# spaceandtimefdn/blitzar

Hardware: NVIDIA H100
Metric: MSM throughput (scalar*point terms/sec), ristretto255, n=2^20 per GPU (higher is better)
Workload: dtype u32 limbs (integer modular arithmetic)

## Files before the change

blitzar_b200/csrc/msm.cuh:

```cuda
#pragma once
#include <algorithm>
#include <vector>

#include "batch_affine.cuh"
#include "curve.cuh"
#include "engine_api.cuh"
#include "lanefield.cuh"

namespace b200 {

struct ColumnDesc {
  const unsigned char* base;
  u64 row_stride;
  u32 bit_offset;
  u32 bit_width;
  u32 n;
  u32 is_signed;
  u32 first_window;
  u32 num_windows;
  u32 table_n;
  u32 gen_base;
};
B200_HD u32 bucket_windows(const ColumnDesc& col) { return col.table_n ? (col.num_windows ? 1u : 0u) : col.num_windows; }

B200_HD void load_scalar_bits(u32 v[8], bool& negative, const ColumnDesc& col, u64 i) {
  const unsigned char* row = col.base + i * col.row_stride;
#pragma unroll
  for (int k = 0; k < 8; ++k)
    v[k] = 0;
  const u32 width = col.bit_width;
  const unsigned char* p = row + (col.bit_offset >> 3);
  const u32 sh = col.bit_offset & 7u;
  if (sh == 0 && width == 256 && (((size_t)p) & 15u) == 0) {
    const uint4* q = (const uint4*)p;
    uint4 a = q[0], b = q[1];
    v[0] = a.x; v[1] = a.y; v[2] = a.z; v[3] = a.w;
    v[4] = b.x; v[5] = b.y; v[6] = b.z; v[7] = b.w;
  } else if (sh == 0 && (width & 31u) == 0 && (((size_t)p) & 3u) == 0) {
    const u32* q = (const u32*)p;
#pragma unroll
    for (int k = 0; k < 8; ++k)
      if ((u32)k < (width >> 5))
        v[k] = q[k];
  } else {
    const u32 nbytes = (sh + width + 7u) >> 3;
#pragma unroll
    for (int k = 0; k < 8; ++k) {
      u64 acc = 0;
#pragma unroll
      for (int b = 0; b < 5; ++b) {
        u32 idx = 4u * k + b;
        if (idx < nbytes)
          acc |= (u64)p[idx] << (8 * b);
      }
      v[k] = (u32)(acc >> sh);
    }
#pragma unroll
    for (int k = 0; k < 8; ++k) {
      int lo = 32 * k;
      if ((int)width <= lo)
        v[k] = 0;
      else if ((int)width < lo + 32)
        v[k] &= (1u << (width - lo)) - 1u;
    }
  }
  negative = false;
  if (col.is_signed) {
    u32 top = width - 1;
    bool neg = false;
#pragma unroll
    for (int k = 0; k < 8; ++k)
      if ((top >> 5) == (u32)k)
        neg = (v[k] >> (top & 31u)) & 1u;
    if (neg) {
      u64 c = 1;
#pragma unroll
      for (int k = 0; k < 8; ++k) {
        int lo = 32 * k;
        u32 m = 0;
        if ((int)width >= lo + 32)
          m = 0xffffffffu;
        else if ((int)width > lo)
          m = (1u << (width - lo)) - 1u;
        c += (u64)((~v[k]) & m);
        v[k] = (u32)c & m;
        c = (m == 0xffffffffu) ? (c >> 32) : 0;
      }
      negative = true;
    }
  }
}

constexpr u32 kAllWindows = 0xffffffffu;
template <class Fn>
B200_HD void for_each_digit(const u32 v[8], bool negative, const ColumnDesc& col, u32 c,
                            u32 nbuckets, Fn f, u32 only_window = kAllWindows) {
  const u32 half = nbuckets;
  const u32 mask = (1u << c) - 1u;
  u64 buf = 0;
  u32 nb = 0, w = 0, carry = 0;
  const u32 W = only_window == kAllWindows
                    ? col.num_windows
                    : (only_window < col.num_windows ? only_window + 1 : 0u);
#pragma unroll
  for (int k = 0; k < 8; ++k) {
    buf |= (u64)v[k] << nb;
    nb += 32;
    while (nb >= c && w < W) {
      u32 d = ((u32)buf & mask) + carry;
      buf >>= c;
      nb -= c;
      bool dneg = d > half;
      carry = dneg ? 1u : 0u;
      if (dneg)
        d = (1u << c) - d;
      if (d && (only_window == kAllWindows || w == only_window))
        f((col.first_window + (col.table_n ? 0u : w)) * nbuckets + (d - 1u), negative != dneg, w);
      ++w;
    }
  }
  while (w < W) {
    u32 d = ((u32)buf & mask) + carry;
    buf >>= c;
    bool dneg = d > half;
    carry = dneg ? 1u : 0u;
    if (dneg)
      d = (1u << c) - d;
    if (d && (only_window == kAllWindows || w == only_window))
      f((col.first_window + (col.table_n ? 0u : w)) * nbuckets + (d - 1u), negative != dneg, w);
    ++w;
  }
}

B200_HD u32 column_of(const u64* col_start, u32 ncols, u64 tid) {
  u32 lo = 0, hi = ncols;
  while (hi - lo > 1) {
    const u32 mid = (lo + hi) >> 1;
    if (tid >= col_start[mid])
      lo = mid;
    else
      hi = mid;
  }
  return lo;
}
struct CountBody {
  static constexpr int kBlock = 256;
  const ColumnDesc* cols;
  const u64* col_start;
  u32 ncols, c, nbuckets;
  u32* counts;
  B200_HD void operator()(u64 tid) const {
    const u32 j = column_of(col_start, ncols, tid);
    const ColumnDesc col = cols[j];
    u64 i = tid - col_start[j];
    u32 v[8];
    bool neg;
    load_scalar_bits(v, neg, col, i);
    u32* cnt = counts;
    for_each_digit(v, neg, col, c, nbuckets, [cnt](u32 key, bool, u32) { B200_ATOMIC_ADD(&cnt[key], 1u); });
  }
};

struct ScatterBody {
  static constexpr int kBlock = 256;
  const ColumnDesc* cols;
  const u64* col_start;
  u32 ncols, c, nbuckets;
  u32* cursor;
  u64* entries;
  u64 total_terms;
  B200_HD void operator()(u64 tid) const {
    u32 only = kAllWindows;
    if (total_terms) {
      only = (u32)(tid / total_terms);
      tid -= (u64)only * total_terms;
    }
    const u32 j = column_of(col_start, ncols, tid);
    const ColumnDesc col = cols[j];
    if (only != kAllWindows && only >= col.num_windows)
      return;
    u64 i = tid - col_start[j];
    u32 v[8];
    bool neg;
    load_scalar_bits(v, neg, col, i);
    u32* cur = cursor;
    u64* en = entries;
    const u32 ii = (u32)i + col.gen_base, tn = col.table_n;
    for_each_digit(v, neg, col, c, nbuckets, [cur, en, ii, tn](u32 key, bool negate, u32 w) {
      u32 pos = B200_ATOMIC_ADD(&cur[key], 1u);
      en[pos] = ((u64)key << 32) | (u64)(((ii + w * tn) << 1) | (negate ? 1u : 0u));
    }, only);
  }
};

constexpr u32 kScanChunk = 256, kScanChunkFirst = 64;
struct ScanUpBody {
  static constexpr int kBlock = 128;
  const u32* in;
  u64 n;
  u32* partial;
  u32 chunk;
  B200_HD void operator()(u64 t) const {
    u64 b = t * chunk, e = b + chunk < n ? b + chunk : n;
    u32 s = 0;
    for (u64 i = b; i < e; ++i)
      s += in[i];
    partial[t] = s;
  }
};
struct ScanTopBody {
  static constexpr int kBlock = 32;
  u32* data;
  u64 n;
  B200_HD void operator()(u64) const {
    u32 s = 0;
    for (u64 i = 0; i < n; ++i) {
      u32 v = data[i];
      data[i] = s;
      s += v;
    }
  }
};
struct ScanDownBody {
  static constexpr int kBlock = 128;
  u32* data;
  u64 n;
  const u32* partial_scanned;
  u32 chunk;
  B200_HD void operator()(u64 t) const {
    u64 b = t * chunk, e = b + chunk < n ? b + chunk : n;
    u32 s = partial_scanned[t];
    for (u64 i = b; i < e; ++i) {
      u32 v = data[i];
      data[i] = s;
      s += v;
    }
  }
};

inline void exclusive_scan(u32* data, u64 n, stream_t s, u32 chunk = kScanChunkFirst) {
  if (n <= kScanChunk) {
    launch(ScanTopBody{data, n}, 1, s);
    return;
  }
  u64 m = (n + chunk - 1) / chunk;
  u32* partial = (u32*)dev_alloc(m * sizeof(u32), s);
  launch(ScanUpBody{data, n, partial, chunk}, m, s);
  exclusive_scan(partial, m, s, kScanChunk);
  launch(ScanDownBody{data, n, partial, chunk}, m, s);
  dev_free(partial, s);
}

#if defined(__CUDACC__) && !defined(B200_EMULATE)
#define B200_BINNED_SORT 1
constexpr u32 kMicroBins = 16384, kBinCap = 8192, kBinSpan = 4096, kMaxBinShift = 12;
constexpr u64 kBinnedSortMinEntries = 1ull << 20;

template <int kBlock> __device__ u32 block_exclusive_scan(u32 v, u32* warp_sums, u32* total) {
  const u32 lane = threadIdx.x & 31u, warp = threadIdx.x >> 5;
  u32 x = v;
#pragma unroll
  for (int d = 1; d < 32; d <<= 1) {
    const u32 y = __shfl_up_sync(0xffffffffu, x, d);
    if (lane >= (u32)d)
      x += y;
  }
  if (lane == 31)
    warp_sums[warp] = x;
  __syncthreads();
  if (warp == 0) {
    u32 w = lane < kBlock / 32 ? warp_sums[lane] : 0u;
#pragma unroll
    for (int d = 1; d < 32; d <<= 1) {
      const u32 y = __shfl_up_sync(0xffffffffu, w, d);
      if (lane >= (u32)d)
        w += y;
    }
    if (lane < kBlock / 32)
      warp_sums[lane] = w;
  }
  __syncthreads();
  const u32 pre = (warp ? warp_sums[warp - 1] : 0u) + x - v;
  *total = warp_sums[kBlock / 32 - 1];
  __syncthreads();
  return pre;
}

template <class Fn>
__device__ void for_each_entry(const ColumnDesc* cols, const u64* col_start, u32 ncols, u32 c,
                               u32 nbuckets, u64 tid, Fn f) {
  const u32 j = column_of(col_start, ncols, tid);
  const ColumnDesc col = cols[j];
  const u64 i = tid - col_start[j];
  u32 v[8];
  bool neg;
  load_scalar_bits(v, neg, col, i);
  const u32 ii = (u32)i + col.gen_base, tn = col.table_n;
  for_each_digit(v, neg, col, c, nbuckets, [&](u32 key, bool negate, u32 w) {
    f(key, ((u64)key << 32) | (u64)(((ii + w * tn) << 1) | (negate ? 1u : 0u)));
  });
}

struct MicroCountBody {
  static constexpr int kBlock = 512;
  const ColumnDesc* cols;
  const u64* col_start;
  u32 ncols, c, nbuckets;
  u64 total_terms;
  u32 tile, shift, nmicro;
  u32* micro_counts;
  __device__ void run(u32 b, unsigned char* smem) const {
    u32* h = (u32*)smem;
    for (u32 m = threadIdx.x; m < nmicro; m += kBlock)
      h[m] = 0;
    __syncthreads();
    const u64 lo = (u64)b * tile, hi = lo + tile < total_terms ? lo + tile : total_terms;
    const u32 sh = shift;
    for (u64 t = lo + threadIdx.x; t < hi; t += kBlock)
      for_each_entry(cols, col_start, ncols, c, nbuckets, t,
                     [h, sh](u32 key, u64) { atomicAdd(&h[key >> sh], 1u); });
    __syncthreads();
    for (u32 m = threadIdx.x; m < nmicro; m += kBlock)
      if (h[m])
        atomicAdd(&micro_counts[m], h[m]);
  }
};

struct PlanBinsBody {
  static constexpr int kBlock = 1024;
  const u32* micro_counts;
  u32 nmicro, span_micro;
  u64 nkeys;
  u32* bin_of;
  u32* bin_start;
  u32* bin_micro;
  u32* bin_cursor;
  u32* nbins_out;
  u32* counts;
  u32* d_m;
  __device__ bool starts_bin(const u32* st, u32 m) const {
    constexpr u32 H = kBinCap / 2;
    return m == 0 || m % span_micro == 0 || micro_counts[m] > H || micro_counts[m - 1] > H ||
           st[m] / H != st[m - 1] / H;
  }
  __device__ void run(u32, unsigned char* smem) const {
    __shared__ u32 ws[32];
    u32* st = (u32*)smem;
    const u32 per = (nmicro + kBlock - 1) / kBlock, m0 = min(threadIdx.x * per, nmicro),
              m1 = min(m0 + per, nmicro);
    u32 sum = 0;
    for (u32 m = m0; m < m1; ++m)
      sum += micro_counts[m];
    u32 total;
    u32 run = block_exclusive_scan<kBlock>(sum, ws, &total);
    for (u32 m = m0; m < m1; ++m) {
      st[m] = run;
      run += micro_counts[m];
    }
    __syncthreads();
    u32 nf = 0;
    for (u32 m = m0; m < m1; ++m)
      nf += starts_bin(st, m) ? 1u : 0u;
    u32 nbins;
    u32 id = block_exclusive_scan<kBlock>(nf, ws, &nbins);
    for (u32 m = m0; m < m1; ++m) {
      if (starts_bin(st, m)) {
        bin_start[id] = st[m];
        bin_micro[id] = m;
        bin_cursor[id] = st[m];
        ++id;
      }
      bin_of[m] = id - 1;
    }
    if (threadIdx.x == 0) {
      bin_start[nbins] = total;
      bin_micro[nbins] = nmicro;
      *nbins_out = nbins;
      counts[nkeys] = total;
      d_m[0] = total;
    }
  }
};

struct CoarseScatterBody {
  static constexpr int kBlock = 1024;
  const ColumnDesc* cols;
  const u64* col_start;
  u32 ncols, c, nbuckets;
  u64 total_terms;
  u32 tile, shift, nmicro;
  const u32* bin_of;
  const u32* nbins_ptr;
  u32* bin_cursor;
  u64* tmp;
  __device__ void run(u32 b, unsigned char* smem) const {
    __shared__ u32 ws[32];
    u32* h = (u32*)smem;
    u32* delta = h + nmicro;
    u64* stage = (u64*)(delta + nmicro + (nmicro & 1u));
    const u32 nbins = *nbins_ptr;
    for (u32 k = threadIdx.x; k < nbins; k += kBlock)
      h[k] = 0;
    __syncthreads();
    const u64 lo = (u64)b * tile, hi = lo + tile < total_terms ? lo + tile : total_terms;
    const u32 sh = shift;
    const u32* map = bin_of;
    for (u64 t = lo + threadIdx.x; t < hi; t += kBlock)
      for_each_entry(cols, col_start, ncols, c, nbuckets, t,
                     [h, sh, map](u32 key, u64) { atomicAdd(&h[__ldg(&map[key >> sh])], 1u); });
    __syncthreads();
    const u32 per = (nbins + kBlock - 1) / kBlock, k0 = min(threadIdx.x * per, nbins),
              k1 = min(k0 + per, nbins);
    u32 sum = 0;
    for (u32 k = k0; k < k1; ++k)
      sum += h[k];
    u32 size;
    u32 run = block_exclusive_scan<kBlock>(sum, ws, &size);
    for (u32 k = k0; k < k1; ++k) {
      const u32 n = h[k];
      if (n)
        delta[k] = atomicAdd(&bin_cursor[k], n) - run;
      h[k] = run;
      run += n;
    }
    __syncthreads();
    for (u64 t = lo + threadIdx.x; t < hi; t += kBlock)
      for_each_entry(cols, col_start, ncols, c, nbuckets, t, [h, sh, map, stage](u32 key, u64 e) {
        stage[atomicAdd(&h[__ldg(&map[key >> sh])], 1u)] = e;
      });
    __syncthreads();
    for (u32 i = threadIdx.x; i < size; i += kBlock) {
      const u64 e = stage[i];
      tmp[delta[__ldg(&map[(u32)(e >> 32) >> sh])] + i] = e;
    }
  }
};

struct BinSortBody {
  static constexpr int kBlock = 1024;
  static constexpr size_t kSmem = 2 * kBinCap * sizeof(u64) + kBinSpan * sizeof(u32);
  const u64* tmp;
  const u32* bin_start;
  const u32* bin_micro;
  const u32* nbins_ptr;
  u32 shift;
  u64 nkeys;
  u64* entries;
  u32* counts;
  __device__ void run(u32 b, unsigned char* smem) const {
    __shared__ u32 ws[32];
    if (b >= *nbins_ptr)
      return;
    u64* ent = (u64*)smem;
    u32* h = (u32*)(smem + 2 * kBinCap * sizeof(u64));
    const u32 lo = bin_start[b], size = bin_start[b + 1] - lo;
    const u64 klo = (u64)bin_micro[b] << shift, khi_m = (u64)bin_micro[b + 1] << shift;
    const u32 span = (u32)((khi_m < nkeys ? khi_m : nkeys) - klo);
    const bool local = size <= kBinCap;
    for (u32 k = threadIdx.x; k < span; k += kBlock)
      h[k] = 0;
    if (local) {
#pragma unroll 4
      for (u32 i = threadIdx.x; i < size; i += kBlock)
        ent[i] = tmp[(u64)lo + i];
    }
    __syncthreads();
    for (u32 i = threadIdx.x; i < size; i += kBlock) {
      const u64 e = local ? ent[i] : tmp[(u64)lo + i];
      atomicAdd(&h[(u32)(e >> 32) - (u32)klo], 1u);
    }
    __syncthreads();
    const u32 per = (span + kBlock - 1) / kBlock, k0 = min(threadIdx.x * per, span),
              k1 = min(k0 + per, span);
    u32 sum = 0;
    for (u32 k = k0; k < k1; ++k)
      sum += h[k];
    u32 total;
    u32 run = block_exclusive_scan<kBlock>(sum, ws, &total);
    for (u32 k = k0; k < k1; ++k) {
      const u32 n = h[k];
      h[k] = run;
      run += n;
      counts[klo + k] = lo + run;
    }
    __syncthreads();
    if (!local) {
      for (u32 i = threadIdx.x; i < size; i += kBlock) {
        const u64 e = tmp[(u64)lo + i];
        entries[(u64)lo + atomicAdd(&h[(u32)(e >> 32) - (u32)klo], 1u)] = e;
      }
      return;
    }
    u64* sorted = ent + kBinCap;
    for (u32 i = threadIdx.x; i < size; i += kBlock) {
      const u64 e = ent[i];
      sorted[atomicAdd(&h[(u32)(e >> 32) - (u32)klo], 1u)] = e;
    }
    __syncthreads();
    for (u32 i = threadIdx.x; i < size; i += kBlock)
      entries[(u64)lo + i] = sorted[i];
  }
};

inline u32 binned_sort_shift(u64 nkeys) {
  u32 shift = 0;
  while ((nkeys + (1ull << shift) - 1) >> shift > kMicroBins)
    ++shift;
  return shift;
}

inline void binned_sort(stream_t s, const ColumnDesc* d_cols, const u64* d_col_start, u32 ncols,
                        u32 c, u32 nbuckets, u64 total_terms, u64 max_entries, u32 max_windows,
                        u64 nkeys, u64* entries, u32* counts, u32* d_m) {
  const u32 shift = binned_sort_shift(nkeys);
  const u32 nmicro = (u32)((nkeys + (1ull << shift) - 1) >> shift);
  const u32 span_micro = std::max(1u, kBinSpan >> shift);
  u32* ws = (u32*)dev_alloc((5ull * nmicro + 3) * sizeof(u32), s);
  u32 *micro_counts = ws, *bin_of = ws + nmicro, *bin_cursor = ws + 2ull * nmicro,
      *bin_start = ws + 3ull * nmicro, *bin_micro = ws + 4ull * nmicro + 1,
      *nbins = ws + 5ull * nmicro + 2;
  u64* tmp = (u64*)dev_alloc(std::max<u64>(max_entries, 1) * sizeof(u64), s);
  dev_zero(micro_counts, nmicro * sizeof(u32), s);
  const u64 count_tile = 4096;
  launch_blocks(MicroCountBody{d_cols, d_col_start, ncols, c, nbuckets, total_terms,
                               (u32)count_tile, shift, nmicro, micro_counts},
                (total_terms + count_tile - 1) / count_tile, nmicro * sizeof(u32), s);
  launch_blocks(PlanBinsBody{micro_counts, nmicro, span_micro, nkeys, bin_of, bin_start, bin_micro,
                             bin_cursor, nbins, counts, d_m},
                1, nmicro * sizeof(u32), s);
  const size_t scatter_smem = 220 * 1024;
  const size_t bin_bytes = (2ull * nmicro + 2) * sizeof(u32);
  const u64 stage_entries = (scatter_smem - bin_bytes) / sizeof(u64);
  const u64 scatter_tile = std::max<u64>(1, stage_entries / max_windows);
  launch_blocks(CoarseScatterBody{d_cols, d_col_start, ncols, c, nbuckets, total_terms,
                                  (u32)scatter_tile, shift, nmicro, bin_of, nbins, bin_cursor, tmp},
                (total_terms + scatter_tile - 1) / scatter_tile, scatter_smem, s);
  launch_blocks(BinSortBody{tmp, bin_start, bin_micro, nbins, shift, nkeys, entries, counts}, nmicro,
                BinSortBody::kSmem, s);
  dev_free(tmp, s);
  dev_free(ws, s);
}
#endif

template <class C> struct FillIdentityBody {
  static constexpr int kBlock = 256;
  static constexpr u32 kChunks = sizeof(typename C::Point) / 16;
  static_assert(sizeof(typename C::Point) % 16 == 0, "points are made of 16-byte aligned fields");
  uint4* p;
  B200_HD void operator()(u64 t) const {
    const typename C::Point id = C::identity();
    const u32 k = (u32)(t % kChunks);
    uint4 v = ((const uint4*)&id)[0];
#pragma unroll
    for (u32 j = 1; j < kChunks; ++j)
      if (j == k)
        v = ((const uint4*)&id)[j];
    p[t] = v;
  }
};
template <class C> inline void fill_identity(stream_t s, typename C::Point* p, u64 n) {
  launch(FillIdentityBody<C>{(uint4*)p}, n * FillIdentityBody<C>::kChunks, s);
}

template <class C> struct MergeBucketsBody {
  static constexpr int kBlock = 128;
  const u32* bucket_end;
  const u32* bucket_begin;
  const typename C::Point* scratch;
  typename C::Point* buckets;
  B200_HD void operator()(u64 k) const {
    const u32 lo = bucket_begin ? bucket_begin[k] : (k ? bucket_end[k - 1] : 0u);
    if (bucket_end[k] == lo)
      return;
    typename C::Point b = buckets[k];
    C::add(b, b, scratch[k]);
    buckets[k] = b;
  }
};

template <class C, bool kGather, class X = SeqExec, bool kUniform = false, bool kUnitZ = false>
struct AccumulateBody {
  static constexpr int kBlock = 128;
  static constexpr int kMinBlocks = !kGather ? 1 : (C::F::N > 8 ? 2 : 3);
  typedef typename C::Point Point;
  typedef typename C::Gen Gen;
  const u32* keys;
  const u64* entries;
  const Gen* gens;
  const Point* pieces;
  const u32* m_ptr;
  u32 K;
  u32 final_level;
  Point* buckets;
  u32* out_keys;
  Point* out_pieces;
  u32* out_m_ptr;
  const u32* unit_veto;

  B200_HD void put_bucket(u32 key, const Point& acc, bool writer) const {
    if (writer)
      buckets[key] = acc;
  }
  B200_HD u32 key_at(u64 i) const { return kGather ? (u32)(entries[i] >> 32) : keys[i]; }
  B200_HD void fetch(Point& acc, u64 i, bool first) const {
    if (kGather) {
      u32 e = (u32)entries[i];
      if (first)
        C::gen_to_point(acc, gens[e >> 1], e & 1u);
      else
        C::template add_gen<X>(acc, acc, gens[e >> 1], e & 1u);
    } else {
      if (first)
        acc = pieces[i];
      else
        C::template add<X>(acc, acc, pieces[i]);
    }
  }
  template <bool kUnit> B200_HD Gen load_gen(u32 idx) const {
    if constexpr (kUnit)
      return C::load_unit_gen(gens + idx);
    else
      return gens[idx];
  }
  template <bool kUnit>
  B200_HD void gather_walk(u64 t, u64 b, u64 e, bool writer, u32& cur, Point& acc,
                           bool& first_seg) const {
    u64 ent = entries[b];
    Gen g = load_gen<kUnit>((u32)ent >> 1);
    cur = (u32)(ent >> 32);
    struct {
      Point p;
      B200_HD void start(const Gen& g, bool negate) { C::gen_to_point(p, g, negate); }
      B200_HD void add(const Gen& g, bool negate) {
        C::template add_gen<X>(p, p, g, negate, kUnit);
      }
      B200_HD void get(Point& out) const { out = p; }
    } ga;
    for (u64 i = b; i < e; ++i) {
      u64 ent_n = ent;
      Gen g_n = g;
      if (i + 1 < e) {
        ent_n = entries[i + 1];
        g_n = load_gen<kUnit>((u32)ent_n >> 1);
      }
      const u32 k = (u32)(ent >> 32);
      const bool negate = ((u32)ent & 1u) != 0;
      if (kUniform) {
        if (i == b) {
          ga.p = C::identity();
        } else if (k != cur) {
          ga.get(acc);
          if (final_level || !first_seg) {
            put_bucket(cur, acc, writer);
          } else if (writer) {
            out_keys[2 * t] = cur;
            out_pieces[2 * t] = acc;
          }
          first_seg = false;
          cur = k;
          ga.p = C::identity();
        }
        ga.add(g, negate);
      } else if (i == b) {
        ga.start(g, negate);
      } else if (k == cur) {
        ga.add(g, negate);
      } else {
        ga.get(acc);
        if (final_level || !first_seg) {
          put_bucket(cur, acc, writer);
        } else if (writer) {
          out_keys[2 * t] = cur;
          out_pieces[2 * t] = acc;
        }
        first_seg = false;
        cur = k;
        ga.start(g, negate);
      }
      ent = ent_n;
      g = g_n;
    }
    ga.get(acc);
  }
  B200_HD void operator()(u64 tid) const {
    const u64 t = tid / X::kLanes;
    const bool writer = (tid % X::kLanes) == 0;
    const u64 M = *m_ptr;
    const u64 T = (M + K - 1) / K;
    if (tid == 0 && out_m_ptr)
      *out_m_ptr = final_level ? 0u : (u32)(2 * T);
    u64 b = t * K;
    if (b >= M)
      return;
    u64 e = b + K < M ? b + K : M;
    u32 cur;
    Point acc;
    bool first_seg = true;
    if (kGather) {
      if (kUnitZ && unit_veto && *unit_veto)
        gather_walk<false>(t, b, e, writer, cur, acc, first_seg);
      else
        gather_walk<kUnitZ>(t, b, e, writer, cur, acc, first_seg);
    } else {
      cur = key_at(b);
      fetch(acc, b, true);
      for (u64 i = b + 1; i < e; ++i) {
        u32 k = key_at(i);
        if (k == cur) {
          fetch(acc, i, false);
        } else {
          if (final_level || !first_seg) {
            put_bucket(cur, acc, writer);
          } else if (writer) {
            out_keys[2 * t] = cur;
            out_pieces[2 * t] = acc;
          }
          first_seg = false;
          cur = k;
          fetch(acc, i, true);
        }
      }
    }
    if (final_level) {
      put_bucket(cur, acc, writer);
      return;
    }
    if (!writer)
      return;
    if (first_seg) {
      out_keys[2 * t] = cur;
      out_pieces[2 * t] = acc;
      out_keys[2 * t + 1] = cur;
      out_pieces[2 * t + 1] = C::identity();
    } else {
      out_keys[2 * t + 1] = cur;
      out_pieces[2 * t + 1] = acc;
    }
  }
};

struct WindowUsedBody {
  static constexpr int kBlock = 64;
  const u32* bucket_end;
  u32 nbuckets;
  u32* window_used;
  B200_HD void operator()(u64 w) const {
    u32 lo = w ? bucket_end[w * nbuckets - 1] : 0u;
    u32 hi = bucket_end[(w + 1) * nbuckets - 1];
    if (hi != lo)
      window_used[w] = 1u;
  }
};

struct WindowUsedFromCountsBody {
  static constexpr int kBlock = 128;
  const u32* counts;
  u64 nkeys;
  u32 nbuckets;
  u32* window_used;
  B200_HD void operator()(u64 t) const {
    const u64 b = t * 256, e = b + 256 < nkeys ? b + 256 : nkeys;
    for (u64 k = b; k < e; ++k)
      if (counts[k])
        window_used[k / nbuckets] = 1u;
  }
};

template <class C, class Ex = SeqExec> struct ReduceBody {
  static constexpr int kBlock = 64;
  typedef typename C::Point Point;
  const Point* X;
  const Point* Cin;
  u32 m_in, g, log2g;
  Point* Xout;
  Point* Cout;
  const u32* window_used;
  u32 nbuckets;
  B200_HD void operator()(u64 tid) const {
    const u64 t = tid / Ex::kLanes;
    const bool writer = (tid % Ex::kLanes) == 0;
    const u32 m_out = m_in / g;
    const u32 w = (u32)(t / m_out), k = (u32)(t % m_out);
    if (window_used[w] == 0) {
      if (writer) {
        Xout[t] = C::identity();
        Cout[t] = C::identity();
      }
      return;
    }
    const Point* x = X + (u64)w * m_in + (u64)k * g;
    Point run = x[g - 1];
    Point acc = Cin ? C::identity() : run;
    if (Cin) {
      acc = run;
      if (g == 1)
        acc = C::identity();
    }
    for (u32 r = g - 1; r-- > 0;) {
      C::template add<Ex>(run, run, x[r]);
      if (r > 0 || !Cin)
        C::template add<Ex>(acc, acc, run);
    }
    if (Cin) {
      const Point* cin = Cin + (u64)w * m_in + (u64)k * g;
      for (u32 r = 0; r < g; ++r)
        C::template add<Ex>(acc, acc, cin[r]);
    }
    for (u32 i = 0; i < log2g; ++i)
      C::template dbl<Ex>(run, run);
    if (writer) {
      Xout[t] = run;
      Cout[t] = acc;
    }
  }
};

template <class C, class X = SeqExec> struct CombineBody {
  static constexpr int kBlock = 32;
  typedef typename C::Point Point;
  const Point* S;
  const ColumnDesc* cols;
  u32 c;
  Point* out;
  B200_HD void operator()(u64 tid) const {
    const u64 j = tid / X::kLanes;
    const bool writer = (tid % X::kLanes) == 0;
    const ColumnDesc col = cols[j];
    if (col.num_windows == 0 || col.n == 0) {
      if (writer)
        out[j] = C::identity();
      return;
    }
    const u32 nw = bucket_windows(col);
    Point acc = S[col.first_window + nw - 1];
    for (u32 w = nw - 1; w-- > 0;) {
      for (u32 i = 0; i < c; ++i)
        C::template dbl<X>(acc, acc);
      C::template add<X>(acc, acc, S[col.first_window + w]);
    }
    if (writer)
      out[j] = acc;
  }
};

#if defined(__CUDACC__) && !defined(B200_EMULATE)
#define B200_LANE_TAIL 1
struct CombineLaneBody {
  static constexpr int kBlock = 32;
  typedef Ed25519 C;
  const C::Point* S;
  const ColumnDesc* cols;
  u32 c;
  C::Point* out;
  __device__ void operator()(u64 tid) const {
    const u64 j = tid >> 5;
    const ColumnDesc col = cols[j];
    if (col.num_windows == 0 || col.n == 0) {
      if ((tid & 31u) == 0)
        out[j] = C::identity();
      return;
    }
    const lane10::Lane L = lane10::lane_info();
    const u32 nw = bucket_windows(col);
    C::Point acc = S[col.first_window + nw - 1];
    for (u32 w = nw - 1; w-- > 0;) {
      u32 t;
      const u32 v = lane10::dbl_n(L, lane10::slice_point(L, acc), (int)c, t);
      lane10::gather_point(acc, v, t);
      C::add<QuadExecConv>(acc, acc, S[col.first_window + w]);
    }
    if ((tid & 31u) == 0)
      out[j] = acc;
  }
};
struct LanePow {
  static __device__ __forceinline__ void pow22523(F25519::E& r, const F25519::E& a) {
    const lane10::Lane L = lane10::lane_info();
    const u32 g = L.base / 10u;
    lane10::gather(r, lane10::pow22523(L, lane10::slice(L, a)), g < 3 ? g : 0u);
  }
};
struct StoreLaneBody {
  static constexpr int kBlock = 32;
  const Ed25519::Point* pts;
  unsigned char* out;
  u64 count;
  __device__ void operator()(u64 tid) const {
    const u32 lane = (u32)tid & 31u, g = lane / 10u;
    const u64 i = (tid >> 5) * 3 + g;
    const bool live = g < 3 && i < count;
    unsigned char enc[32];
    Ed25519::encode<LanePow>(enc, pts[live ? i : count - 1]);
    if (live && lane == 10u * g) {
      uint4* d = (uint4*)(out + 32 * i);
      const uint4* e = (const uint4*)enc;
      d[0] = e[0];
      d[1] = e[1];
    }
  }
};
#endif

template <class C>
inline void launch_store_commit(stream_t s, const typename C::Point* pts, unsigned char* out,
                                u64 count, bool lane_tail = true);

template <class C, bool kProjective> struct IngestBody {
  static constexpr int kBlock = 128;
  const unsigned char* raw;
  typename C::Gen* gens;
  B200_HD void operator()(u64 i) const {
    typename C::Gen g;
    if (kProjective)
      C::load_proj_abi(g, raw + i * C::kAbiProjBytes);
    else
      C::load_gen_abi(g, raw + i * C::kAbiGenBytes);
    gens[i] = g;
  }
};
constexpr int kMaxTableWindows = 33;
template <class C> struct PrecomputeTableBody {
  static constexpr int kBlock = 64;
  typename C::Gen* table;
  u64 n;
  u32 c, W;
  B200_HD void operator()(u64 i) const {
    typedef typename C::F F;
    typename C::Point p, pts[kMaxTableWindows];
    typename F::E prefix[kMaxTableWindows], acc = F::one(), inv;
    C::gen_to_point(p, table[i], false);
    for (u32 w = 0; w < W; ++w) {
      if (w)
        for (u32 k = 0; k < c; ++k)
          C::dbl(p, p);
      pts[w] = p;
      prefix[w] = acc;
      F::mul(acc, acc, C::denominator(p));
    }
    F::invert(inv, acc);
    for (u32 w = W; w-- > 0;) {
      typename F::E zi;
      F::mul(zi, inv, prefix[w]);
      F::mul(inv, inv, C::denominator(pts[w]));
      typename C::Gen g;
      C::normalized_gen(g, pts[w], zi);
      table[(u64)w * n + i] = g;
    }
  }
};
template <class C> struct IngestCompactBody {
  static constexpr int kBlock = 128;
  const unsigned char* table;
  u32 window_width;
  typename C::Gen* gens;
  B200_HD void operator()(u64 i) const {
    const u64 group = i / window_width, j = i % window_width;
    const u64 entry = (group << window_width) + (1ull << j);
    typename C::Gen g;
    C::load_compact_abi(g, table + entry * C::kAbiCompactBytes);
    gens[i] = g;
  }
};
struct BuiltinGeneratorBody {
  static constexpr int kBlock = 64;
  Ed25519::Gen* gens;
  u64 first;
  B200_HD void operator()(u64 i) const {
    Ed25519::Point g;
    Ed25519::builtin_generator(g, first + i);
    Ed25519::point_to_gen(gens[i], g);
  }
};
struct GenPieces {
  const u64* start;
  const u64* from;
  const u64* to;
  u32 npieces;
};
template <class C> struct IngestPiecesBody {
  static constexpr int kBlock = IngestBody<C, false>::kBlock;
  const unsigned char* raw;
  typename C::Gen* gens;
  GenPieces p;
  B200_HD void operator()(u64 tid) const {
    const u32 k = column_of(p.start, p.npieces, tid);
    IngestBody<C, false>{raw + p.from[k] * C::kAbiGenBytes, gens + p.to[k]}(tid - p.start[k]);
  }
};
struct BuiltinPiecesBody {
  static constexpr int kBlock = BuiltinGeneratorBody::kBlock;
  Ed25519::Gen* gens;
  GenPieces p;
  B200_HD void operator()(u64 tid) const {
    const u32 k = column_of(p.start, p.npieces, tid);
    BuiltinGeneratorBody{gens + p.to[k], p.from[k]}(tid - p.start[k]);
  }
};

struct IngestMap {
  GenPieces p;
  B200_HD void at(u64 i, u64& src, u64& dst) const {
    if (p.npieces == 0) {
      src = dst = i;
      return;
    }
    const u32 k = column_of(p.start, p.npieces, i);
    src = p.from[k] + (i - p.start[k]);
    dst = p.to[k] + (i - p.start[k]);
  }
};
constexpr u32 kNormBlock = 256;
struct NormalizeUpBody {
  static constexpr int kBlock = 128;
  typedef F25519 F;
  const unsigned char* raw;
  IngestMap map;
  u64 n, T;
  F::E* pre;
  F::E* prod;
  u32* invalid;
  B200_HD F::E group(u64 j) const {
    F::E z[kBatchGroup], acc = F::one();
#pragma unroll
    for (u32 k = 0; k < kBatchGroup; ++k) {
      const u64 i = j + k * T;
      z[k] = F::one();
      if (i < n) {
        u64 src, dst;
        map.at(i, src, dst);
        z[k] = Ed25519::load_abi_z(raw + src * Ed25519::kAbiGenBytes);
      }
    }
#pragma unroll
    for (u32 k = 0; k < kBatchGroup; ++k) {
      const u64 i = j + k * T;
      if (i >= n)
        break;
      if (F::is_zero(z[k])) {
        *invalid = 1u;
        z[k] = F::one();
      }
      pre[i] = acc;
      F::mul(acc, acc, z[k]);
    }
    return acc;
  }
  B200_HD void operator()(u64 j) const { prod[j] = group(j); }
};
struct NormalizeDownBody {
  static constexpr int kBlock = 128;
  typedef F25519 F;
  const unsigned char* raw;
  IngestMap map;
  u64 n, T;
  const F::E* pre;
  const F::E* prod;
  const F::E* ps;
  const u32* invalid;
  Ed25519::Gen* gens;
  B200_HD void operator()(u64 j) const {
    const bool scale = *invalid == 0;
    F::E inv = prod[ps ? j / kNormBlock : j];
    if (ps)
      F::mul(inv, inv, ps[j]);
    for (u32 k = kBatchGroup; k-- > 0;) {
      const u64 i = j + k * T;
      if (i >= n)
        continue;
      u64 src, dst;
      map.at(i, src, dst);
      Ed25519::Point p;
      Ed25519::load_point_abi(p, raw + src * Ed25519::kAbiGenBytes);
      if (scale) {
        F::E zi;
        F::mul(zi, inv, pre[i]);
        F::mul(inv, inv, p.Z);
        F::mul(p.X, p.X, zi);
        F::mul(p.Y, p.Y, zi);
        F::mul(p.T, p.T, zi);
        p.Z = F::one();
      }
      Ed25519::Gen g;
      Ed25519::point_to_gen(g, p);
      gens[dst] = g;
    }
  }
};
#ifdef B200_BINNED_SORT
__device__ __forceinline__ F25519::E shfl_up_fe(const F25519::E& a, u32 d) {
  F25519::E r;
#pragma unroll
  for (int k = 0; k < 8; ++k)
    r.l[k] = __shfl_up_sync(0xffffffffu, a.l[k], d);
  return r;
}
__device__ __forceinline__ F25519::E shfl_down_fe(const F25519::E& a, u32 d) {
  F25519::E r;
#pragma unroll
  for (int k = 0; k < 8; ++k)
    r.l[k] = __shfl_down_sync(0xffffffffu, a.l[k], d);
  return r;
}
template <int kBlock>
__device__ void block_prefix_suffix(const F25519::E& x, F25519::E& P, F25519::E& S,
                                    F25519::E& total, F25519::E* ws) {
  typedef F25519 F;
  const u32 lane = threadIdx.x & 31u, warp = threadIdx.x >> 5;
  F::E inc = x, sinc = x;
#pragma unroll
  for (u32 d = 1; d < 32; d <<= 1) {
    const F::E y = shfl_up_fe(inc, d), z = shfl_down_fe(sinc, d);
    if (lane >= d)
      F::mul(inc, inc, y);
    if (lane + d < 32)
      F::mul(sinc, sinc, z);
  }
  F::E pe = shfl_up_fe(inc, 1), se = shfl_down_fe(sinc, 1);
  if (lane == 0)
    pe = F::one();
  if (lane == 31) {
    se = F::one();
    ws[warp] = inc;
  }
  __syncthreads();
  F::E before = F::one(), after = F::one();
  for (u32 w = 0; w < kBlock / 32; ++w) {
    if (w < warp)
      F::mul(before, before, ws[w]);
    else if (w > warp)
      F::mul(after, after, ws[w]);
  }
  F::mul(P, before, pe);
  F::mul(S, se, after);
  F::mul(total, before, ws[warp]);
  F::mul(total, total, after);
  __syncthreads();
}
struct NormalizeUpBlockBody {
  static constexpr int kBlock = kNormBlock;
  typedef F25519 F;
  NormalizeUpBody up;
  F::E* ps;
  F::E* prod;
  __device__ void run(u32 b, unsigned char*) const {
    __shared__ F::E ws[kBlock / 32];
    const u64 j = (u64)b * kBlock + threadIdx.x;
    const F::E g = j < up.T ? up.group(j) : F::one();
    F::E P, S, total;
    block_prefix_suffix<kBlock>(g, P, S, total, ws);
    if (j < up.T)
      F::mul(ps[j], P, S);
    if (threadIdx.x == 0)
      prod[b] = total;
  }
};
struct NormalizeMidBody {
  static constexpr int kBlock = 1024;
  typedef F25519 F;
  F::E* vals;
  F::E* pre;
  u64 m;
  __device__ void run(u32, unsigned char*) const {
    __shared__ F::E ws[kBlock / 32];
    __shared__ F::E inv_total;
    const u64 per = (m + kBlock - 1) / kBlock, lo = min((u64)threadIdx.x * per, m),
              hi = min(lo + per, m);
    F::E c = F::one();
    for (u64 k = lo; k < hi; ++k) {
      pre[k] = c;
      F::mul(c, c, vals[k]);
    }
    F::E P, S, total;
    block_prefix_suffix<kBlock>(c, P, S, total, ws);
    if (threadIdx.x == 0)
      F::invert(inv_total, total);
    __syncthreads();
    F::E inv;
    F::mul(inv, inv_total, P);
    F::mul(inv, inv, S);
    for (u64 k = hi; k-- > lo;) {
      const F::E v = vals[k];
      F::mul(vals[k], inv, pre[k]);
      F::mul(inv, inv, v);
    }
  }
};
#endif
inline void ingest_normalized(stream_t s, const unsigned char* raw, Ed25519::Gen* gens,
                              const IngestMap& map, u64 n, u32* invalid) {
  typedef F25519::E fe;
  if (n == 0)
    return;
  const u64 T = (n + kBatchGroup - 1) / kBatchGroup;
  fe* pre = (fe*)dev_alloc(n * sizeof(fe), s);
  const NormalizeUpBody up{raw, map, n, T, pre, nullptr, invalid};
#ifdef B200_BINNED_SORT
  const u64 blocks = (T + kNormBlock - 1) / kNormBlock;
  fe* ps = (fe*)dev_alloc((T + 2 * blocks) * sizeof(fe), s);
  fe* prod = ps + T;
  launch_blocks(NormalizeUpBlockBody{up, ps, prod}, blocks, 0, s);
  launch_blocks(NormalizeMidBody{prod, prod + blocks, blocks}, 1, 0, s);
  launch(NormalizeDownBody{raw, map, n, T, pre, prod, ps, invalid, gens}, T, s);
  dev_free(ps, s);
#else
  fe* prod = (fe*)dev_alloc(T * sizeof(fe), s);
  NormalizeUpBody u = up;
  u.prod = prod;
  launch(u, T, s);
  batch_invert<F25519>(s, prod, T);
  launch(NormalizeDownBody{raw, map, n, T, pre, prod, nullptr, invalid, gens}, T, s);
  dev_free(prod, s);
#endif
  dev_free(pre, s);
}
template <class C, bool kCommit> struct StoreBody {
  static constexpr int kBlock = 32;
  const typename C::Point* pts;
  unsigned char* out;
  B200_HD void operator()(u64 i) const {
    if (kCommit)
      C::store_commit_abi(out + i * C::kAbiCommitBytes, pts[i]);
    else
      C::store_proj_abi(out + i * C::kAbiProjBytes, pts[i]);
  }
};
template <class C>
inline void launch_store_commit(stream_t s, const typename C::Point* pts, unsigned char* out,
                                u64 count, bool lane_tail) {
#ifdef B200_LANE_TAIL
  if constexpr (C::kCurveId == kRistretto255) {
    if (lane_tail && count && count <= 4096) {
      launch(StoreLaneBody{pts, out, count}, (count + 2) / 3 * 32, s);
      return;
    }
  }
#endif
  launch(StoreBody<C, true>{pts, out}, count, s);
}
template <class C> struct GenToProjBody {
  static constexpr int kBlock = 64;
  const typename C::Gen* gens;
  unsigned char* out;
  B200_HD void operator()(u64 i) const {
    typename C::Point p;
    C::gen_to_point(p, gens[i], false);
    C::store_proj_abi(out + i * C::kAbiProjBytes, p);
  }
};
template <class C> struct SumPartsBody {
  static constexpr int kBlock = 32;
  const typename C::Point* parts;
  u32 nparts, count;
  typename C::Point* out;
  B200_HD void operator()(u64 j) const {
    typename C::Point acc = parts[j];
    for (u32 r = 1; r < nparts; ++r)
      C::add(acc, acc, parts[(u64)r * count + j]);
    out[j] = acc;
  }
};

inline u32 choose_window_bits(u64 max_n, u32 max_width, u32 ncols, size_t point_bytes) {
  const double kMaxBucketBytes = 3.0e9;
  u32 best = 2;
  double best_cost = 1e300;
  for (u32 c = 2; c <= 16; ++c) {
    double W = (double)(max_width / c + 1);
    if (c > 8 && W * (double)(1u << (c - 1)) * (double)ncols * (double)point_bytes > kMaxBucketBytes)
      break;
    double cost = W * ((double)max_n + 2.5 * (double)(1u << (c - 1)));
    if (cost < best_cost) {
      best_cost = cost;
      best = c;
    }
  }
  return best;
}

struct MsmPlan {
  u32 c = 0, nbuckets = 0, ncols = 0, total_windows = 0;
  u64 nkeys = 0, max_n = 0, total_terms = 0, total_entries = 0;
  std::vector<ColumnDesc> cols;
};

inline MsmPlan msm_make_plan(std::vector<ColumnDesc> cols, const MsmOptions& opt,
                             size_t point_bytes) {
  MsmPlan p;
  p.ncols = (u32)cols.size();
  u32 max_width = 1;
  for (auto& col : cols) {
    p.max_n = std::max<u64>(p.max_n, col.n);
    p.total_terms += col.n;
    if (col.n)
      max_width = std::max(max_width, col.bit_width);
  }
  p.c = opt.window_bits ? opt.window_bits
                        : choose_window_bits(p.max_n, max_width, p.ncols, point_bytes);
  p.nbuckets = 1u << (p.c - 1);
  u64 max_entries = 0;
  for (auto& col : cols) {
    col.first_window = p.total_windows;
    col.num_windows = col.n ? col.bit_width / p.c + 1 : 0;
    p.total_windows += bucket_windows(col);
    max_entries += (u64)col.n * col.num_windows;
    if (col.table_n)
      B200_REQUIRE((u64)col.table_n * col.num_windows < (1ull << 31), "generator table too large");
    if (col.n)
      B200_REQUIRE((u64)col.gen_base + col.n + (u64)(col.num_windows - 1) * col.table_n < (1ull << 31),
                   "generator index of a column too large");
  }
  p.nkeys = (u64)p.total_windows * p.nbuckets;
  p.total_entries = max_entries;
  B200_REQUIRE(p.nkeys < (1ull << 32), "too many buckets for one pass");
  p.cols = std::move(cols);
  return p;
}

struct StagedRange {
  const ColumnDesc* d_cols = nullptr;
  const u64* d_col_start = nullptr;
  u64 total_terms = 0, max_entries = 0;
  u32 max_windows = 0;
  StagedRange(stream_t s, const MsmPlan& plan, u64 begin, u64 end) {
    const u32 ncols = plan.ncols;
    std::vector<ColumnDesc> cols(plan.cols);
    std::vector<u64> col_start(ncols + 1, 0);
    for (u32 j = 0; j < ncols; ++j) {
      u64 lo = std::min<u64>(begin, cols[j].n), hi = std::min<u64>(end, cols[j].n);
      cols[j].base += lo * cols[j].row_stride;
      cols[j].n = (u32)(hi - lo);
      col_start[j + 1] = col_start[j] + cols[j].n;
      max_entries += (u64)cols[j].n * cols[j].num_windows;
      max_windows = std::max(max_windows, cols[j].n ? cols[j].num_windows : 0u);
    }
    total_terms = col_start[ncols];
    if (total_terms == 0)
      return;
    B200_REQUIRE(max_entries < (1ull << 32) && end - begin < (1ull << 31),
                 "too many (term, window) entries for one sort pass");
    const size_t desc_bytes = ncols * sizeof(ColumnDesc), start_bytes = (ncols + 1) * sizeof(u64);
    std::vector<unsigned char> stage(desc_bytes + start_bytes);
    std::memcpy(stage.data(), cols.data(), desc_bytes);
    std::memcpy(stage.data() + desc_bytes, col_start.data(), start_bytes);
    d_cols = (const ColumnDesc*)stage_to_device(s, stage.data(), stage.size());
    d_col_start = (const u64*)((const unsigned char*)d_cols + desc_bytes);
  }
};

struct SortedLayout {
  u64* entries;
  u32* counts;
  u32* starts;
  u32* d_m;
  u64 slots_max;
  bool binned;
};

inline SortedLayout sort_entries(stream_t s, const MsmPlan& plan, const StagedRange& r, u32 L,
                                 const MsmOptions& opt, u32* window_used) {
  const u32 ncols = plan.ncols, c = plan.c, nbuckets = plan.nbuckets;
  const u64 nkeys = plan.nkeys, max_entries = r.max_entries, total_terms = r.total_terms;
  SortedLayout out{};
  out.slots_max = L ? ((max_entries + nkeys * ((1ull << L) - 1) + (1ull << L) - 1) >> L) << L : max_entries;
  out.counts = (u32*)dev_alloc((nkeys + 1) * sizeof(u32), s);
  out.d_m = (u32*)dev_alloc(16 * sizeof(u32), s);
  out.entries = (u64*)dev_alloc(out.slots_max * sizeof(u64), s);
#ifdef B200_BINNED_SORT
  out.binned = L == 0 && opt.sort_path != 0 && binned_sort_shift(nkeys) <= kMaxBinShift &&
               (opt.sort_path == 2 || max_entries >= kBinnedSortMinEntries);
  if (out.binned)
    binned_sort(s, r.d_cols, r.d_col_start, ncols, c, nbuckets, total_terms, max_entries,
                r.max_windows, nkeys, out.entries, out.counts, out.d_m);
#endif
  if (!out.binned) {
    dev_zero(out.counts, (nkeys + 1) * sizeof(u32), s);
    launch(CountBody{r.d_cols, r.d_col_start, ncols, c, nbuckets, out.counts}, total_terms, s);
    if (L) {
      launch(WindowUsedFromCountsBody{out.counts, nkeys, nbuckets, window_used}, (nkeys + 255) / 256, s);
      launch(PadCountsBody{out.counts, (1u << L) - 1u}, nkeys, s);
    }
    exclusive_scan(out.counts, nkeys + 1, s);
    copy_d2d(out.d_m, out.counts + nkeys, sizeof(u32), s);
    if (L) {
      out.starts = (u32*)dev_alloc((nkeys + 1) * sizeof(u32), s);
      copy_d2d(out.starts, out.counts, (nkeys + 1) * sizeof(u32), s);
    }
    const bool window_major = opt.scatter_window_major && r.max_windows > 1;
    launch(ScatterBody{r.d_cols, r.d_col_start, ncols, c, nbuckets, out.counts, out.entries,
                       window_major ? total_terms : 0},
           window_major ? total_terms * r.max_windows : total_terms, s);
  }
  if (L)
    launch(FillPadsBody{out.starts, out.counts, out.entries}, nkeys, s);
  else
    launch(WindowUsedBody{out.counts, nbuckets, window_used}, plan.total_windows, s);
  return out;
}

inline unsigned sort_selftest(stream_t s, std::vector<ColumnDesc> cols, u32 c) {
  MsmOptions opt;
  opt.window_bits = c;
  const MsmPlan plan = msm_make_plan(std::move(cols), opt, 160);
  const StagedRange r(s, plan, 0, plan.max_n);
  if (r.total_terms == 0)
    return ~0u;
  const u64 nkeys = plan.nkeys, M = r.max_entries;
  DevBuf<u32> window_used(plan.total_windows, s);
  opt.sort_path = 0;
  const SortedLayout a = sort_entries(s, plan, r, 0, opt, window_used.p);
  opt.sort_path = 2;
  const SortedLayout b = sort_entries(s, plan, r, 0, opt, window_used.p);
  std::vector<u32> ca(nkeys + 1), cb(nkeys + 1), m(1);
  std::vector<u64> ea(M), eb(M);
  copy_d2h(ca.data(), a.counts, (nkeys + 1) * sizeof(u32), s);
  copy_d2h(cb.data(), b.counts, (nkeys + 1) * sizeof(u32), s);
  copy_d2h(m.data(), b.d_m, sizeof(u32), s);
  copy_d2h(ea.data(), a.entries, M * sizeof(u64), s);
  copy_d2h(eb.data(), b.entries, M * sizeof(u64), s);
  stream_sync(s);
  for (void* p : {(void*)a.entries, (void*)a.counts, (void*)a.d_m, (void*)b.entries, (void*)b.counts,
                  (void*)b.d_m, (void*)r.d_cols})
    dev_free(p, s);
  if (!b.binned)
    return ~0u;
  unsigned bad = m[0] == ca[nkeys] ? 0u : 1u;
  for (u64 k = 0; k < nkeys; ++k) {
    const u32 lo = k ? ca[k - 1] : 0u, hi = ca[k];
    if (cb[k] != hi || hi < lo || hi > M) {
      ++bad;
      continue;
    }
    std::sort(ea.begin() + lo, ea.begin() + hi);
    std::sort(eb.begin() + lo, eb.begin() + hi);
    if (!std::equal(ea.begin() + lo, ea.begin() + hi, eb.begin() + lo))
      ++bad;
  }
  return bad;
}

struct RangeHook {
  virtual void before_range(u64 begin, u64 end) = 0;
  virtual void before_accumulate() {}
  virtual ~RangeHook() {}
};

template <class C>
stream_t chunk_walk(stream_t s, stream_t tail, WalkInput<C> walk, u32* d_m, bool unit,
                    const u32* unit_veto, typename C::Point* target, const MsmOptions& opt,
                    std::vector<void*>& to_free) {
  typedef typename C::Point Point;
  u32 K = opt.chunk1 ? std::max(opt.chunk1, 4u) : (walk.m_max >= (1ull << 23) ? 64u : 32u);
  const u32 chunkn = std::max(opt.chunkn, 4u);
  const u32* lvl_keys = nullptr;
  const Point* lvl_pieces = nullptr;
  stream_t cs = s;
  for (int level = 0;; ++level) {
    const bool final_level = walk.m_max <= K;
    u64 T = (walk.m_max + K - 1) / K;
    u32* out_keys = final_level ? nullptr : (u32*)dev_alloc(2 * T * sizeof(u32), cs);
    Point* out_pieces = final_level ? nullptr : (Point*)dev_alloc(2 * T * sizeof(Point), cs);
    to_free.insert(to_free.end(), {out_keys, out_pieces});
    u32* out_m = d_m + 1 + (level % 8);
    if (level == 0) {
      const bool uniform =
          opt.uniform_add == 2 ? C::kCurveId == kRistretto255 : opt.uniform_add != 0;
      constexpr bool kEd = C::kCurveId == kRistretto255;
      const bool unit_path = kEd && unit;
      if (uniform && unit_path)
        launch(AccumulateBody<C, true, SeqExec, true, kEd>{nullptr, walk.entries, walk.gens, nullptr,
                                                            walk.m_ptr, K, final_level, target,
                                                            out_keys, out_pieces, out_m, unit_veto},
               T, s);
      else if (uniform)
        launch(AccumulateBody<C, true, SeqExec, true>{nullptr, walk.entries, walk.gens, nullptr,
                                                      walk.m_ptr, K, final_level, target, out_keys,
                                                      out_pieces, out_m, nullptr},
               T, s);
      else if (unit_path)
        launch(AccumulateBody<C, true, SeqExec, false, kEd>{nullptr, walk.entries, walk.gens, nullptr,
                                                             walk.m_ptr, K, final_level, target,
                                                             out_keys, out_pieces, out_m, unit_veto},
               T, s);
      else
        launch(AccumulateBody<C, true>{nullptr, walk.entries, walk.gens, nullptr, walk.m_ptr, K,
                                       final_level, target, out_keys, out_pieces, out_m, nullptr},
               T, s);
      KernelTimer::get().end(s);
      if (tail != s)
        stream_follow(tail, s);
      cs = tail;
    } else if (T <= opt.quad_threshold) {
      launch(AccumulateBody<C, false, QuadExec>{lvl_keys, nullptr, nullptr, lvl_pieces, walk.m_ptr,
                                                K, final_level, target, out_keys, out_pieces, out_m,
                                                nullptr},
             T * QuadExec::kLanes, cs);
    } else {
      launch(AccumulateBody<C, false>{lvl_keys, nullptr, nullptr, lvl_pieces, walk.m_ptr, K,
                                      final_level, target, out_keys, out_pieces, out_m, nullptr},
             T, cs);
    }
    if (final_level)
      break;
    lvl_keys = out_keys;
    lvl_pieces = out_pieces;
    walk.m_ptr = out_m;
    walk.m_max = 2 * T;
    K = chunkn;
  }
  return cs;
}

template <class C>
void msm_accumulate_range(stream_t s, const MsmPlan& plan, const typename C::Gen* gens, u64 begin,
                          u64 end, bool add_into, typename C::Point* d_buckets,
                          u32* d_window_used, const MsmOptions& opt, stream_t tail,
                          RangeHook* hook = nullptr) {
  const StagedRange r(s, plan, begin, end);
  if (r.total_terms == 0)
    return;
  gens += begin;
  StageRange nvtx_sort("msm: digit count + scan + scatter");
  const u64 max_entries = r.max_entries, nkeys = plan.nkeys;
  u32 L = 0;
  if constexpr (C::kBatchAffine) {
    const double mean = (double)max_entries / (double)nkeys;
    if (opt.pair_levels >= 0)
      L = (u32)opt.pair_levels;
    else if (max_entries >= (1ull << 23))
      while (L < 6 && (double)(32u << L) <= mean)
        ++L;
    while (L > 0 && max_entries + nkeys * ((1ull << L) - 1) >= (1ull << 32) - (1ull << L))
      --L;
  }
  const SortedLayout sorted = sort_entries(s, plan, r, L, opt, d_window_used);
  B200_LOG(3, "range [%llu, %llu): %llu terms, %llu entries max, c=%u, %llu keys, pair levels %u",
           (unsigned long long)begin, (unsigned long long)end, (unsigned long long)r.total_terms,
           (unsigned long long)max_entries, plan.c, (unsigned long long)nkeys, L);
  WalkInput<C> walk{gens, sorted.entries, sorted.d_m, max_entries};
  std::vector<void*> to_free;
  if (hook)
    hook->before_accumulate();
  KernelTimer::get().begin(s);
  StageRange nvtx_acc("msm: bucket accumulation");
  if constexpr (C::kBatchAffine) {
    if (L) {
      walk = run_pair_levels<C>(s, L, sorted.entries, gens, sorted.d_m, sorted.slots_max,
                                opt.pair_batch);
      to_free = {(void*)walk.gens, (void*)walk.entries};
    }
  }
  typedef typename C::Point Point;
  Point* target = add_into ? (Point*)dev_alloc(nkeys * sizeof(Point), s) : d_buckets;
  const bool unit = walk.gens == gens && opt.gens_normalized;
  const stream_t cs =
      chunk_walk<C>(s, tail, walk, sorted.d_m, unit, opt.unit_veto, target, opt, to_free);
  if (add_into) {
    launch(MergeBucketsBody<C>{sorted.counts, sorted.starts, target, d_buckets}, nkeys, cs);
    dev_free(target, cs);
  }
  to_free.insert(to_free.end(), {sorted.d_m, sorted.counts, sorted.starts});
  for (void* ptr : to_free)
    dev_free(ptr, cs);
  dev_free(sorted.entries, s);
  dev_free((void*)r.d_cols, s);
}

template <class C>
void msm_finish(stream_t s, const MsmPlan& plan, const typename C::Point* d_buckets,
                const u32* d_window_used, typename C::Point* out, const MsmOptions& opt) {
  typedef typename C::Point Point;
  StageRange nvtx_fin("msm: bucket reduction + window combination");
  const u32 total_windows = plan.total_windows, nbuckets = plan.nbuckets, ncols = plan.ncols;
  ColumnDesc* d_cols =
      (ColumnDesc*)stage_to_device(s, plan.cols.data(), ncols * sizeof(ColumnDesc));
  Point* d_S = nullptr;
  u32 m = nbuckets;
  const Point* X = d_buckets;
  const Point* Cin = nullptr;
  std::vector<void*> to_free;
  if (m == 1) {
    d_S = (Point*)dev_alloc(total_windows * sizeof(Point), s);
    copy_d2d(d_S, d_buckets, total_windows * sizeof(Point), s);
  }
  bool first = true;
  while (m > 1) {
    u32 g = first ? std::min<u32>(opt.reduce_g1, m) : std::min<u32>(opt.reduce_gn, m);
    u32 log2g = 0;
    while ((1u << log2g) < g)
      ++log2g;
    u32 m_out = m / g;
    Point* Xout = (Point*)dev_alloc((u64)total_windows * m_out * sizeof(Point), s);
    Point* Cout = (Point*)dev_alloc((u64)total_windows * m_out * sizeof(Point), s);
    if ((u64)total_windows * m_out <= opt.quad_threshold)
      launch(ReduceBody<C, QuadExecConv>{X, Cin, m, g, log2g, Xout, Cout, d_window_used, nbuckets},
             (u64)total_windows * m_out * QuadExec::kLanes, s);
    else
      launch(ReduceBody<C>{X, Cin, m, g, log2g, Xout, Cout, d_window_used, nbuckets},
             (u64)total_windows * m_out, s);
    to_free.push_back(Xout);
    if (m_out > 1)
      to_free.push_back(Cout);
    X = Xout;
    Cin = Cout;
    m = m_out;
    first = false;
    if (m == 1)
      d_S = Cout;
  }
  for (void* ptr : to_free)
    dev_free(ptr, s);
  bool uniform_windows = true;
  for (u32 j = 1; j < ncols; ++j)
    uniform_windows = uniform_windows && bucket_windows(plan.cols[j]) == bucket_windows(plan.cols[0]);
#ifdef B200_LANE_TAIL
  bool lane_done = false;
  if constexpr (C::kCurveId == kRistretto255) {
    if (ncols <= 2048 && opt.lane_tail) {
      launch(CombineLaneBody{d_S, d_cols, plan.c, out}, (u64)ncols * 32, s);
      lane_done = true;
    }
  }
  if (lane_done) {
  } else
#endif
  if (ncols <= opt.quad_threshold && uniform_windows)
    launch(CombineBody<C, QuadExecConv>{d_S, d_cols, plan.c, out}, (u64)ncols * QuadExec::kLanes,
           s);
  else if (ncols <= opt.quad_threshold)
    launch(CombineBody<C, QuadExec>{d_S, d_cols, plan.c, out}, (u64)ncols * QuadExec::kLanes, s);
  else
    launch(CombineBody<C>{d_S, d_cols, plan.c, out}, ncols, s);
  dev_free(d_S, s);
  dev_free(d_cols, s);
}

template <class C>
void msm_run(stream_t s, const typename C::Gen* gens, std::vector<ColumnDesc> cols,
             typename C::Point* out, const MsmOptions& opt = MsmOptions(), u32 num_ranges = 1,
             RangeHook* hook = nullptr, stream_t tail = stream_t()) {
  typedef typename C::Point Point;
  if (cols.empty())
    return;
  MsmPlan plan = msm_make_plan(std::move(cols), opt, sizeof(Point));
  B200_LOG(2, "msm: curve %u, %u columns, longest %llu, %llu terms, window %u bits, %u bucket sets%s",
           C::kCurveId, plan.ncols, (unsigned long long)plan.max_n,
           (unsigned long long)plan.total_terms, plan.c, plan.total_windows,
           plan.ncols && plan.cols[0].table_n ? " (fixed-base table)" : "");
  if (plan.total_terms == 0 || plan.total_windows == 0) {
    if (hook)
      hook->before_range(0, plan.max_n);
    fill_identity<C>(s, out, plan.ncols);
    return;
  }
  Point* d_buckets = (Point*)dev_alloc(plan.nkeys * sizeof(Point), s);
  fill_identity<C>(s, d_buckets, plan.nkeys);
  u32* d_window_used = (u32*)dev_alloc(plan.total_windows * sizeof(u32), s);
  dev_zero(d_window_used, plan.total_windows * sizeof(u32), s);
  if (num_ranges < 1)
    num_ranges = 1;
  const u64 limit = opt.max_range_entries ? opt.max_range_entries : (1ull << 31);
  const u64 needed = (plan.total_entries + limit - 1) / limit;
  if (needed > num_ranges)
    num_ranges = (u32)std::min<u64>(needed, plan.max_n);
  const bool overlap = num_ranges > 1 && tail != stream_t() && tail != s;
  for (u32 r = 0; r < num_ranges; ++r) {
    u64 begin = range_begin(plan.max_n, r, num_ranges, opt.range_skew),
        end = range_begin(plan.max_n, r + 1, num_ranges, opt.range_skew);
    if (hook)
      hook->before_range(begin, end);
    msm_accumulate_range<C>(s, plan, gens, begin, end, r > 0, d_buckets, d_window_used, opt,
                            overlap ? tail : s, hook);
  }
  if (overlap)
    stream_follow(s, tail);
  msm_finish<C>(s, plan, d_buckets, d_window_used, out, opt);
  dev_free(d_window_used, s);
  dev_free(d_buckets, s);
}

}
```

Before: 338.1 million.

## Write chunk-local bucket runs directly and merge short split runs in a pass

```diff
diff --git a/blitzar_b200/csrc/msm.cuh b/blitzar_b200/csrc/msm.cuh
--- a/blitzar_b200/csrc/msm.cuh
+++ b/blitzar_b200/csrc/msm.cuh
@@ -578,6 +578,8 @@
   }
 };
 
+constexpr u32 kNullKey = 0xFFFFFFFFu;
+
 template <class C, bool kGather, class X = SeqExec, bool kUniform = false, bool kUnitZ = false>
 struct AccumulateBody {
   static constexpr int kBlock = 128;
@@ -601,6 +603,17 @@
     if (writer)
       buckets[key] = acc;
   }
+  B200_HD void close_run(u64 t, u32 key, const Point& acc, bool writer, bool first_seg,
+                         bool head_open) const {
+    if (final_level || !first_seg || !head_open) {
+      put_bucket(key, acc, writer);
+      if (first_seg && !final_level && writer)
+        out_keys[2 * t] = kNullKey;
+    } else if (writer) {
+      out_keys[2 * t] = key;
+      out_pieces[2 * t] = acc;
+    }
+  }
   B200_HD u32 key_at(u64 i) const { return kGather ? (u32)(entries[i] >> 32) : keys[i]; }
   B200_HD void fetch(Point& acc, u64 i, bool first) const {
     if (kGather) {
@@ -623,7 +636,7 @@
       return gens[idx];
   }
   template <bool kUnit>
-  B200_HD void gather_walk(u64 t, u64 b, u64 e, bool writer, u32& cur, Point& acc,
+  B200_HD void gather_walk(u64 t, u64 b, u64 e, bool writer, bool head_open, u32& cur, Point& acc,
                            bool& first_seg) const {
     u64 ent = entries[b];
     Gen g = load_gen<kUnit>((u32)ent >> 1);
@@ -650,12 +663,7 @@
           ga.p = C::identity();
         } else if (k != cur) {
           ga.get(acc);
-          if (final_level || !first_seg) {
-            put_bucket(cur, acc, writer);
-          } else if (writer) {
-            out_keys[2 * t] = cur;
-            out_pieces[2 * t] = acc;
-          }
+          close_run(t, cur, acc, writer, first_seg, head_open);
           first_seg = false;
           cur = k;
           ga.p = C::identity();
@@ -667,12 +675,7 @@
         ga.add(g, negate);
       } else {
         ga.get(acc);
-        if (final_level || !first_seg) {
-          put_bucket(cur, acc, writer);
-        } else if (writer) {
-          out_keys[2 * t] = cur;
-          out_pieces[2 * t] = acc;
-        }
+        close_run(t, cur, acc, writer, first_seg, head_open);
         first_seg = false;
         cur = k;
         ga.start(g, negate);
@@ -696,30 +699,36 @@
     u32 cur;
     Point acc;
     bool first_seg = true;
+    const bool head_open = !kGather || (b > 0 && key_at(b - 1) == key_at(b));
     if (kGather) {
       if (kUnitZ && unit_veto && *unit_veto)
-        gather_walk<false>(t, b, e, writer, cur, acc, first_seg);
+        gather_walk<false>(t, b, e, writer, head_open, cur, acc, first_seg);
       else
-        gather_walk<kUnitZ>(t, b, e, writer, cur, acc, first_seg);
+        gather_walk<kUnitZ>(t, b, e, writer, head_open, cur, acc, first_seg);
     } else {
-      cur = key_at(b);
-      fetch(acc, b, true);
-      for (u64 i = b + 1; i < e; ++i) {
-        u32 k = key_at(i);
-        if (k == cur) {
+      bool any = false;
+      for (u64 i = b; i < e; ++i) {
+        const u32 k = key_at(i);
+        if (k == kNullKey)
+          continue;
+        if (!any) {
+          any = true;
+          cur = k;
+          fetch(acc, i, true);
+        } else if (k == cur) {
           fetch(acc, i, false);
         } else {
-          if (final_level || !first_seg) {
-            put_bucket(cur, acc, writer);
-          } else if (writer) {
-            out_keys[2 * t] = cur;
-            out_pieces[2 * t] = acc;
-          }
+          close_run(t, cur, acc, writer, first_seg, true);
           first_seg = false;
           cur = k;
           fetch(acc, i, true);
         }
       }
+      if (!any) {
+        if (!final_level && writer)
+          out_keys[2 * t] = out_keys[2 * t + 1] = kNullKey;
+        return;
+      }
     }
     if (final_level) {
       put_bucket(cur, acc, writer);
@@ -727,6 +736,24 @@
     }
     if (!writer)
       return;
+    if (kGather) {
+      const bool tail_open = e < M && key_at(e) == cur;
+      const bool lone = first_seg && head_open;
+      if (first_seg) {
+        out_keys[2 * t] = lone ? cur : kNullKey;
+        if (lone)
+          out_pieces[2 * t] = acc;
+      }
+      if (tail_open) {
+        out_keys[2 * t + 1] = cur;
+        out_pieces[2 * t + 1] = lone ? C::identity() : acc;
+      } else {
+        out_keys[2 * t + 1] = kNullKey;
+        if (!lone)
+          put_bucket(cur, acc, writer);
+      }
+      return;
+    }
     if (first_seg) {
       out_keys[2 * t] = cur;
       out_pieces[2 * t] = acc;
@@ -736,6 +763,57 @@
       out_keys[2 * t + 1] = cur;
       out_pieces[2 * t + 1] = acc;
     }
+  }
+};
+
+template <class C> struct MergeSplitBody {
+  static constexpr int kBlock = 128;
+  static constexpr u32 kMaxSpan = 8;
+  const u32* m_ptr;
+  const u32* keys;
+  const typename C::Point* pieces;
+  typename C::Point* buckets;
+  u32* out_keys;
+  u64 nthreads;
+  B200_HD u64 last_chunk(u64 t, u32 k) const {
+    u64 a = t, e = t;
+    while (keys[2 * a] == k) {
+      if (t - a + 1 >= kMaxSpan)
+        return ~0ull;
+      --a;
+    }
+    while (keys[2 * e + 1] == k) {
+      if (e - a + 1 >= kMaxSpan)
+        return ~0ull;
+      ++e;
+    }
+    return e;
+  }
+  B200_HD void operator()(u64 tid) const {
+    const u64 t = nthreads - 1 - tid;
+    if (2 * t + 2 > *m_ptr)
+      return;
+    typedef typename C::Point Point;
+    const u32 k0 = keys[2 * t], k1 = keys[2 * t + 1];
+    const bool starts = k1 != kNullKey && k1 != k0;
+    Point acc, next;
+    if (starts) {
+      acc = pieces[2 * t + 1];
+      next = pieces[2 * t + 2];
+    }
+    const u64 e0 = k0 == kNullKey ? ~0ull : last_chunk(t, k0);
+    const u64 e1 = k1 == kNullKey ? ~0ull : (k1 == k0 ? e0 : last_chunk(t, k1));
+    out_keys[2 * t] = e0 != ~0ull ? kNullKey : k0;
+    out_keys[2 * t + 1] = e1 != ~0ull ? kNullKey : k1;
+    if (!starts || e1 == ~0ull)
+      return;
+    for (u64 u = t + 1;; ++u) {
+      C::add(acc, acc, next);
+      if (u == e1)
+        break;
+      next = pieces[2 * u + 2];
+    }
+    buckets[k1] = acc;
   }
 };
 
@@ -1489,6 +1567,12 @@
       if (tail != s)
         stream_follow(tail, s);
       cs = tail;
+      if (!final_level) {
+        u32* joined_keys = (u32*)dev_alloc(2 * T * sizeof(u32), cs);
+        to_free.push_back(joined_keys);
+        launch(MergeSplitBody<C>{out_m, out_keys, out_pieces, target, joined_keys, T}, T, cs);
+        out_keys = joined_keys;
+      }
     } else if (T <= opt.quad_threshold) {
       launch(AccumulateBody<C, false, QuadExec>{lvl_keys, nullptr, nullptr, lvl_pieces, walk.m_ptr,
                                                 K, final_level, target, out_keys, out_pieces, out_m,
```

Result: faster. 345.8 million (median of 6 runs) (+2.3%).
